# mala-lab/GGAD

Hardware: AMD Instinct MI355X
Metric: training nodes/sec (DGraph-Fin mini-batch GGAD) (higher is better)
Workload: dtype f32; 1 GPU; DGraph-Fin-size synthetic graph, mini-batch GGAD (GCN encoder); nodes=3700550, directed_entries=72953930, feat=17, emb=64, batch=150+50, graph=powerlaw(alpha=2.1,max_degree=2000), chunk_batches=150, hop2=ldsw, overlap=False, dense_cus=0, chain=0, dense_steps=XCD-resident chunk kernel: one launch per chunk on 28 CUs of one XCD, parallelism=dp1, optimizer=adam(lr=1e-3,wd=0.007), batch_streams=the reference's stream

## Files before the change

ggad_amd/csrc/hop2_ldsw.hip:

```cpp
#include <algorithm>
#include <atomic>
#include <climits>
#include <mutex>

#include "common.h"

namespace {

#ifdef GGAD_G2_PROF
struct G2Prof { unsigned long long a[8], t; };
#define G2_ARG , G2Prof &prof
#define G2_PASS , prof
#define G2_MARK(i) do { __builtin_amdgcn_sched_barrier(0); __builtin_amdgcn_s_waitcnt(0); const unsigned long long t_ = wall_clock64(); \
                        prof.a[i] += t_ - prof.t; prof.t = t_; __builtin_amdgcn_sched_barrier(0); } while (0)
#define TC_MARK(i) do { __syncthreads(); if (threadIdx.x == 0) { const unsigned long long t_ = wall_clock64(); tcp[i] += t_ - tct; tct = t_; } } while (0)
#else
#define G2_ARG
#define G2_PASS
#define G2_MARK(i)
#define TC_MARK(i)
#endif

constexpr int SLICE = 256;
constexpr int GRP_W = 10;
constexpr int ITEM_GRAB = 4;

__global__ void __launch_bounds__(256) k_tile_offsets(const int32_t *__restrict__ rowptr, const int32_t *__restrict__ col,
                                                      int64_t n_nodes, int n_tiles, int shift, int32_t *__restrict__ off) {
  const int64_t u = (int64_t)blockIdx.x * blockDim.x + threadIdx.x;
  if (u >= n_nodes) return;
  const int s = rowptr[u], e = rowptr[u + 1];
  int32_t *o = off + u * (n_tiles + 1);
  int t = 0;
  for (int i = s; i < e; ++i) {
    const int tile = col[i] >> shift;
    while (t <= tile) { o[t] = i - s; ++t; }
  }
  while (t <= n_tiles) { o[t] = e - s; ++t; }
}

__global__ void __launch_bounds__(256) k_tm_blocksum(const int32_t *__restrict__ off, int64_t n_nodes, int n_tiles, int32_t *__restrict__ bsum) {
  __shared__ int wsum[4][64];
  const int lane = lane_id(), w = threadIdx.x >> 6;
  const int NT1 = n_tiles + 1;
  const int64_t u0 = (int64_t)blockIdx.x * 256 + 64 * w;
  for (int t0 = 0; t0 < n_tiles; t0 += 64) {
    const int t = t0 + lane;
    int acc = 0;
    if (t < n_tiles)
      for (int i = 0; i < 64 && u0 + i < n_nodes; ++i) { const int32_t *o = off + (u0 + i) * NT1 + t; acc += o[1] - o[0]; }
    wsum[w][lane] = acc;
    __syncthreads();
    if (w == 0 && t < n_tiles) bsum[(int64_t)blockIdx.x * n_tiles + t] = wsum[0][lane] + wsum[1][lane] + wsum[2][lane] + wsum[3][lane];
    __syncthreads();
  }
}

__global__ void __launch_bounds__(1024) k_tm_scan(int32_t *__restrict__ bsum, int64_t n_blocks, int n_tiles, int32_t *__restrict__ tile_base) {
  extern __shared__ int tot[];
  for (int t = threadIdx.x; t < n_tiles; t += blockDim.x) {
    int run = 0;
    int64_t b = 0;
    for (; b + 8 <= n_blocks; b += 8) {
      int v[8];
#pragma unroll
      for (int q = 0; q < 8; ++q) v[q] = bsum[(b + q) * n_tiles + t];
#pragma unroll
      for (int q = 0; q < 8; ++q) { bsum[(b + q) * n_tiles + t] = run; run += v[q]; }
    }
    for (; b < n_blocks; ++b) { const int v = bsum[b * n_tiles + t]; bsum[b * n_tiles + t] = run; run += v; }
    tot[t] = run;
  }
  __syncthreads();
  if (threadIdx.x == 0) {
    int run = 0;
    for (int t = 0; t < n_tiles; ++t) { tile_base[t] = run; run += tot[t]; }
    tile_base[n_tiles] = run;
  }
}

__global__ void __launch_bounds__(256) k_tm_fill(const int32_t *__restrict__ rowptr, const int32_t *__restrict__ col,
                                                 const int32_t *__restrict__ off, int64_t n_nodes, int n_tiles,
                                                 const int32_t *__restrict__ bsum, const int32_t *__restrict__ tile_base,
                                                 int32_t *__restrict__ tile_start, int32_t *__restrict__ col_t) {
  __shared__ int wsum[4][64];
  const int lane = lane_id(), w = threadIdx.x >> 6;
  const int NT1 = n_tiles + 1;
  const int64_t u0 = (int64_t)blockIdx.x * 256 + 64 * w;
  for (int t0 = 0; t0 <= n_tiles; t0 += 64) {
    const int t = t0 + lane;
    int acc = 0;
    if (t < n_tiles)
      for (int i = 0; i < 64 && u0 + i < n_nodes; ++i) { const int32_t *o = off + (u0 + i) * NT1 + t; acc += o[1] - o[0]; }
    wsum[w][lane] = acc;
    __syncthreads();
    if (t < n_tiles) {
      int pos = tile_base[t] + bsum[(int64_t)blockIdx.x * n_tiles + t];
      for (int ww = 0; ww < w; ++ww) pos += wsum[ww][lane];
      for (int i = 0; i < 64 && u0 + i < n_nodes; ++i) {
        const int64_t u = u0 + i;
        const int32_t *o = off + u * NT1 + t;
        const int o0 = o[0], o1 = o[1];
        tile_start[u * NT1 + t] = pos;
        const int32_t *src = col + rowptr[u] + o0;
        for (int j = 0; j < o1 - o0; ++j) col_t[pos + j] = src[j];
        pos += o1 - o0;
      }
    } else if (t == n_tiles) {
      for (int i = 0; i < 64 && u0 + i < n_nodes; ++i) tile_start[(u0 + i) * NT1 + t] = 0;
    }
    __syncthreads();
  }
}

constexpr int TW_SHIFT = 15;
constexpr int TW_TILE = 1 << TW_SHIFT;
constexpr int TW_MAXOWN = 6144;
constexpr int TW_T = 1024;
constexpr int TW_BRK = 1536;

constexpr int TT_SLAB = 128;
__global__ void __launch_bounds__(256) k_seg_transpose(const int32_t *__restrict__ tile_off, const int32_t *__restrict__ tile_start,
                                                       int n_tiles, const int32_t *__restrict__ ent_own,
                                                       const int32_t *__restrict__ ent_col, int n_ents, int64_t seg_stride,
                                                       int32_t *__restrict__ seg_t, int skip) {
  __shared__ int tl[TT_SLAB][65];
  unsigned vbx, vgx;
  if (!ggad_vblock(skip, vbx, vgx)) return;
  const int p0 = vbx * 64;
  if (p0 >= n_ents) return;
  const int lane = lane_id(), wid = threadIdx.x >> 6;
  const int NT1 = n_tiles + 1;
  int u_l = 0, own_l = 0;
  if (p0 + lane < n_ents) { own_l = ent_own[p0 + lane] == p0 + lane ? 1 : 0; u_l = own_l ? ent_col[p0 + lane] : 0; }
  for (int which = 0; which < (tile_start ? 2 : 1); ++which) {
  const int32_t *table = which ? tile_start : tile_off;
  int32_t *plane = seg_t + (which ? (int64_t)NT1 * seg_stride : 0);
  for (int t0 = 0; t0 < NT1; t0 += TT_SLAB) {
    int v0[16], v1[16];
    const int c0 = min(t0 + lane, NT1 - 1), c1 = min(t0 + 64 + lane, NT1 - 1);
#pragma unroll
    for (int jj = 0; jj < 16; ++jj) {
      const int j = wid + 4 * jj;
      const int u = __shfl(u_l, j, GGAD_WAVE);
      const int32_t *row = table + (int64_t)u * NT1;
      v0[jj] = row[c0];
      v1[jj] = row[c1];
    }
#pragma unroll
    for (int jj = 0; jj < 16; ++jj) {
      const int j = wid + 4 * jj;
      const int own = __shfl(own_l, j, GGAD_WAVE);
      if (t0 + lane < NT1) tl[lane][j] = own ? v0[jj] : 0;
      if (t0 + 64 + lane < NT1) tl[64 + lane][j] = own ? v1[jj] : 0;
    }
    __syncthreads();
    const int nt = min(TT_SLAB, NT1 - t0);
    for (int idx = threadIdx.x; idx < nt * 64; idx += 256) {
      const int tt = idx >> 6, j = idx & 63;
      if (p0 + j < n_ents) plane[(int64_t)(t0 + tt) * seg_stride + p0 + j] = tl[tt][j];
    }
    __syncthreads();
  }
  }
}

__device__ __forceinline__ int block_excl_scan_1024(int v, int *warp_buf, int *total) {
  const int lane = lane_id(), wid = threadIdx.x >> 6;
  int inc = v;
#pragma unroll
  for (int off = 1; off < 64; off <<= 1) {
    const int t = __shfl_up(inc, off, 64);
    if (lane >= off) inc += t;
  }
  if (lane == 63) warp_buf[wid] = inc;
  __syncthreads();
  int base = 0, tot = 0;
#pragma unroll
  for (int w = 0; w < 16; ++w) { const int sv = warp_buf[w]; if (w < wid) base += sv; tot += sv; }
  __syncthreads();
  *total = tot;
  return base + inc - v;
}

__global__ void __launch_bounds__(TW_T) k_tile_counts(const int32_t *__restrict__ col, const int32_t *__restrict__ seg_t,
                                                      int64_t n_cap, const int32_t *__restrict__ own_rp,
                                                      const int32_t *__restrict__ batch_ent_ptr,
                                                      const int32_t *__restrict__ pw_base, uint16_t *__restrict__ pc, int n_tiles,
                                                      int n_batches, int32_t *__restrict__ counters, int skip, int tile_major) {
  extern __shared__ __attribute__((aligned(16))) uint32_t lds_u[];
  uint32_t *cnt = lds_u;
  int *offs = reinterpret_cast<int *>(lds_u + TW_TILE / 2);
  int *segbeg = offs + TW_MAXOWN + 1;
  int *dst = segbeg + TW_MAXOWN;
  int *brk = dst + TW_MAXOWN;
  __shared__ int wbuf[16];
  unsigned vbx, vgx;
  if (!ggad_vblock(skip, vbx, vgx)) return;
  int t, b;
  const bool class_map = (tile_major & 2) != 0;
  tile_major &= 1;
  if (class_map) {
    const int nx = skip < 0 ? 8 : 7, c = (int)(blockIdx.x & 7u);
    const int ci = c - ((skip >= 0 && c > skip) ? 1 : 0);
    const unsigned j = blockIdx.x >> 3;
    const int nt_c = ci < n_tiles ? (n_tiles - ci + nx - 1) / nx : 0;
    if (j >= (unsigned)nt_c * (unsigned)n_batches) return;
    t = ci + nx * (int)(j / (unsigned)n_batches);
    b = (int)(j % (unsigned)n_batches);
  } else {
    if (vbx >= (unsigned)n_tiles * (unsigned)n_batches) return;
    t = (int)(vbx % (unsigned)n_tiles); b = (int)(vbx / (unsigned)n_tiles);
  }
  const int o0 = batch_ent_ptr[b], o1 = batch_ent_ptr[b + 1];
  const int n_own_all = o1 - o0;
  const int32_t *seg_lo = seg_t + (int64_t)t * n_cap, *seg_hi = seg_lo + n_cap;
  const int32_t *seg_st = tile_major ? seg_t + (int64_t)(n_tiles + 1 + t) * n_cap : own_rp;
#ifdef GGAD_G2_PROF
  unsigned long long tcp[8] = {0, 0, 0, 0, 0, 0, 0, 0}, tct = wall_clock64();
#endif
  for (int i = threadIdx.x; i < TW_TILE / 2; i += TW_T) cnt[i] = 0u;
  constexpr int IPT = TW_MAXOWN / TW_T;
  const int n_slabs = (n_own_all + TW_MAXOWN - 1) / TW_MAXOWN;
  const bool one_slab = n_slabs == 1;
  constexpr int CACHE_IT = 16;
  int kc[CACHE_IT], dc[CACHE_IT];
  for (int pass = 0; pass < 2; ++pass) {
    for (int slab = 0; slab < n_slabs; ++slab) {
      const int ob0 = o0 + slab * TW_MAXOWN;
      const int n_own = min(TW_MAXOWN, o1 - ob0);
      if (pass == 0 || n_slabs > 1) {
        {
          int lo_[IPT], hi_[IPT], rp_[IPT], pb_[IPT];
#pragma unroll
          for (int q = 0; q < IPT; ++q) {
            const int i = min((int)threadIdx.x + q * TW_T, n_own - 1);
            lo_[q] = seg_lo[ob0 + i]; hi_[q] = seg_hi[ob0 + i]; rp_[q] = seg_st[ob0 + i]; pb_[q] = pw_base[ob0 + i];
          }
#pragma unroll
          for (int q = 0; q < IPT; ++q) {
            const int i = (int)threadIdx.x + q * TW_T;
            if (i < n_own) { offs[i] = hi_[q] - lo_[q]; segbeg[i] = rp_[q] + (tile_major ? 0 : lo_[q]); dst[i] = pb_[q] + lo_[q]; }
          }
        }
        __syncthreads();
        TC_MARK(0);
        int len[IPT];
        int mysum = 0;
#pragma unroll
        for (int q = 0; q < IPT; ++q) {
          const int i = threadIdx.x * IPT + q;
          len[q] = (i < n_own) ? offs[i] : 0;
          mysum += len[q];
        }
        __syncthreads();
        int P0;
        int ex = block_excl_scan_1024(mysum, wbuf, &P0);
#pragma unroll
        for (int q = 0; q < IPT; ++q) {
          const int i = threadIdx.x * IPT + q;
          if (i < n_own) offs[i] = ex;
          ex += len[q];
        }
        if (threadIdx.x == 0) offs[n_own] = P0;
        __syncthreads();
        TC_MARK(1);
      }
      const int P = offs[n_own];
      if (P > 0) {
        const int s0 = 1 << (31 - __clz(n_own));
        auto locate = [&](int pp, int &own, int &j) {
          int lo = 0;
          for (int st = s0; st > 0; st >>= 1) { const int m = lo + st; lo = (offs[min(m, n_own)] <= pp) ? m : lo; }
          own = lo; j = pp - offs[lo];
        };
        const int nblk = ((P - 1) >> 6) + 1;
        const bool use_brk = nblk + 1 <= TW_BRK;
        if (use_brk && (pass == 0 || n_slabs > 1)) {
          for (int b = threadIdx.x; b <= nblk; b += TW_T) {
            int own = n_own, j = 0;
            if (b < nblk) locate(min(64 * b, P - 1), own, j);
            brk[b] = own;
          }
          __syncthreads();
        }
        auto locate4 = [&](const int (&pp)[4], int (&own)[4], int (&j)[4]) {
          int lo[4] = {0, 0, 0, 0};
          int smax = s0;
          if (use_brk) {
            smax = 0;
#pragma unroll
            for (int q = 0; q < 4; ++q) {
              const int b = pp[q] >> 6;
              lo[q] = brk[b];
              const int w = brk[b + 1] - lo[q];
              smax = max(smax, w > 0 ? 1 << (31 - __clz(w)) : 0);
            }
          }
          for (int st = smax; st > 0; st >>= 1) {
#pragma unroll
            for (int q = 0; q < 4; ++q) { const int m = lo[q] + st; lo[q] = (offs[min(m, n_own)] <= pp[q]) ? m : lo[q]; }
          }
#pragma unroll
          for (int q = 0; q < 4; ++q) { own[q] = lo[q]; j[q] = pp[q] - offs[lo[q]]; }
        };
        int p_start = 0;
        if (one_slab) {
          if (pass == 0) {
#pragma unroll
            for (int g4 = 0; g4 < CACHE_IT; g4 += 4) {
              if (g4 * TW_T < P) {
                int pp[4], own[4], j[4];
#pragma unroll
                for (int q = 0; q < 4; ++q) pp[q] = min((g4 + q) * TW_T + (int)threadIdx.x, P - 1);
                locate4(pp, own, j);
#pragma unroll
                for (int q = 0; q < 4; ++q) {
                  kc[g4 + q] = col[segbeg[own[q]] + j[q]];
                  dc[g4 + q] = dst[own[q]] + j[q];
                }
              } else {
#pragma unroll
                for (int q = 0; q < 4; ++q) { kc[g4 + q] = 0; dc[g4 + q] = 0; }
              }
            }
#pragma unroll
            for (int it = 0; it < CACHE_IT; ++it) {
              const bool on = it * TW_T + (int)threadIdx.x < P;
              const int loc = kc[it] & (TW_TILE - 1);
              if (on) atomicAdd(&cnt[loc >> 1], 1u << ((loc & 1) << 4));
              kc[it] = on ? loc : -1;
            }
          } else {
#pragma unroll
            for (int it = 0; it < CACHE_IT; ++it)
              if (kc[it] >= 0) pc[dc[it]] = (uint16_t)((cnt[kc[it] >> 1] >> ((kc[it] & 1) << 4)) & 0xFFFFu);
          }
          p_start = CACHE_IT * TW_T;
          TC_MARK(2 + 2 * pass);
        }
        for (int p0 = p_start; p0 < P; p0 += 4 * TW_T) {
          int pp[4], own[4], j[4];
#pragma unroll
          for (int q = 0; q < 4; ++q) pp[q] = min(p0 + q * TW_T + (int)threadIdx.x, P - 1);
          locate4(pp, own, j);
          int k4[4];
#pragma unroll
          for (int q = 0; q < 4; ++q) k4[q] = col[segbeg[own[q]] + j[q]];
#pragma unroll
          for (int q = 0; q < 4; ++q) {
            if (p0 + q * TW_T + (int)threadIdx.x < P) {
              const int loc = k4[q] & (TW_TILE - 1);
              if (pass == 0) atomicAdd(&cnt[loc >> 1], 1u << ((loc & 1) << 4));
              else pc[(int64_t)dst[own[q]] + j[q]] = (uint16_t)((cnt[loc >> 1] >> ((loc & 1) << 4)) & 0xFFFFu);
            }
          }
        }
        TC_MARK(3 + 2 * pass);
      }
      __syncthreads();
    }
  }
#ifdef GGAD_G2_PROF
  if (threadIdx.x == 0) {
    unsigned long long *out = reinterpret_cast<unsigned long long *>(counters + GGAD_CTR_PROF) + 8;
    for (int k = 0; k < 6; ++k) atomicAdd(out + k, tcp[k]);
    atomicAdd(out + 6, 1ull);
  }
#endif
}

template <int G, int FT>
__device__ __forceinline__ void gather_slice(const int32_t *__restrict__ col, const float *__restrict__ feat, int F_rt, int stride,
                                             int s, int n0, int n1, float inv_sr, int n_occ, const int (&pb)[8],
                                             const uint16_t *__restrict__ pc, int lane, int k_first, float (&tot)[G] G2_ARG) {
  const int F = FT ? FT : F_rt;
  const int rpi = 64 / F;
  const int g = lane / F, f = lane - g * F;
  const bool act = g < rpi;
  const int gl = act ? g : rpi - 1;
  const char *fb = reinterpret_cast<const char *>(feat);
  const uint32_t rs = (uint32_t)stride * 4u, fo = (uint32_t)f * 4u;
  auto row_elem = [&](int kk) -> float { return *reinterpret_cast<const float *>(fb + ((uint32_t)kk * rs + fo)); };
  float acc[G];
#pragma unroll
  for (int j = 0; j < G; ++j) acc[j] = 0.0f;
  const int last = max(n1 - 1, 0);
  int k_nx = k_first;
  uint32_t c_nx[G];
  {
    const int ix = min(n0 + lane, last);
#pragma unroll
    for (int j = 0; j < G; ++j) c_nx[j] = pc[pb[j] + ix];
  }
  G2_MARK(2);
  for (int blk = n0; blk < n1; blk += 64) {
    const bool mine = blk + lane < n1;
    const int k = mine ? k_nx : 0;
    const int count = min(64, n1 - blk);
    float w[G];
    if (FT != 17) {
#pragma unroll
      for (int j = 0; j < G; ++j) w[j] = (j < n_occ && mine) ? inv_sr / sqrtf((float)c_nx[j]) : 0.0f;
    }
    if (FT == 17) {
      constexpr int IT = 22;
      float x[IT];
#pragma unroll
      for (int t = 0; t < IT; ++t) {
        const int kk = __shfl(k, (t * 3 + gl) & 63, GGAD_WAVE);
        x[t] = row_elem(kk);
      }
#pragma unroll
      for (int j = 0; j < G; ++j) w[j] = (j < n_occ && mine) ? inv_sr / sqrtf((float)c_nx[j]) : 0.0f;
      {
        const int ix = min(blk + 64 + lane, last);
        k_nx = col[s + ix];
#pragma unroll
        for (int j = 0; j < G; ++j) c_nx[j] = pc[pb[j] + ix];
      }
      G2_MARK(3);
#pragma unroll
      for (int t = 0; t < IT; ++t) {
        const int src = t * 3 + g;
        const float xv = (act && src < count) ? x[t] : 0.0f;
#pragma unroll
        for (int j = 0; j < G; ++j) {
          const float ws = __shfl(w[j], src & 63, GGAD_WAVE);
          acc[j] = fmaf((src < count) ? ws : 0.0f, xv, acc[j]);
        }
      }
      G2_MARK(4);
    } else {
      const int iters = (count + rpi - 1) / rpi;
      int tt = 0;
      for (; tt + 8 <= iters; tt += 8) {
        float x[8];
#pragma unroll
        for (int q = 0; q < 8; ++q) {
          const int kk = __shfl(k, ((tt + q) * rpi + gl) & 63, GGAD_WAVE);
          x[q] = row_elem(kk);
        }
#pragma unroll
        for (int q = 0; q < 8; ++q) {
          const int src = (tt + q) * rpi + g;
          const float xv = (act && src < count) ? x[q] : 0.0f;
#pragma unroll
          for (int j = 0; j < G; ++j) {
            const float ws = __shfl(w[j], src & 63, GGAD_WAVE);
            acc[j] = fmaf((src < count) ? ws : 0.0f, xv, acc[j]);
          }
        }
      }
      for (; tt < iters; ++tt) {
        const int src = tt * rpi + g;
        const int kk = __shfl(k, (tt * rpi + gl) & 63, GGAD_WAVE);
        const float xr = row_elem(kk);
        const float xv = (act && src < count) ? xr : 0.0f;
#pragma unroll
        for (int j = 0; j < G; ++j) {
          const float ws = __shfl(w[j], src & 63, GGAD_WAVE);
          acc[j] = fmaf((src < count) ? ws : 0.0f, xv, acc[j]);
        }
      }
      const int ix = min(blk + 64 + lane, last);
      k_nx = col[s + ix];
#pragma unroll
      for (int j = 0; j < G; ++j) c_nx[j] = pc[pb[j] + ix];
    }
  }
#pragma unroll
  for (int j = 0; j < G; ++j) {
    float t = acc[j];
    for (int q = 1; q < rpi; ++q) t += __shfl(acc[j], (lane + q * F) & 63, GGAD_WAVE);
    tot[j] = t;
  }
}

constexpr int MF_WS = 68;
constexpr int MF_LDS = 8 * MF_WS + 64;
typedef float mf4 __attribute__((ext_vector_type(4)));
typedef float mf2 __attribute__((ext_vector_type(2)));
typedef int mi4 __attribute__((ext_vector_type(4)));

template <int G>
__device__ __forceinline__ void gather_slice_mfma(const int32_t *__restrict__ col, const float *__restrict__ feat, int s, int n0, int n1,
                                                  float inv_sr, int n_occ, const int (&pb)[8], const uint16_t *__restrict__ pc,
                                                  int lane, float *lw, int k_first, float (&tot)[G] G2_ARG) {
  const int a = lane & 15, g = lane >> 4;
  const char *fb = reinterpret_cast<const char *>(feat) + a * 8;
  int *lids = reinterpret_cast<int *>(lw + 8 * MF_WS);
  const int aa = a < G ? a : 0;
  mf4 acc0 = {0.0f, 0.0f, 0.0f, 0.0f}, acc1 = {0.0f, 0.0f, 0.0f, 0.0f};
  const int last = max(n1 - 1, 0);
  int k_nx = k_first;
  uint32_t c_nx[G];
  {
    const int ix = min(n0 + lane, last);
#pragma unroll
    for (int j = 0; j < G; ++j) c_nx[j] = pc[pb[j] + ix];
  }
  G2_MARK(2);
  for (int blk = n0; blk < n1; blk += 64) {
    const bool mine = blk + lane < n1;
    lids[lane] = k_nx;
    __builtin_amdgcn_fence(__ATOMIC_RELEASE, "wavefront");
    __builtin_amdgcn_wave_barrier();
    int id[16];
#pragma unroll
    for (int c = 0; c < 4; ++c) {
      const mi4 iv = *reinterpret_cast<const mi4 *>(lids + 16 * g + 4 * c);
#pragma unroll
      for (int q = 0; q < 4; ++q) id[4 * c + q] = iv[q];
    }
    mf2 x[16];
#pragma unroll
    for (int i = 0; i < 16; ++i) x[i] = *reinterpret_cast<const mf2 *>(fb + ((uint32_t)id[i] << 7));
#pragma unroll
    for (int j = 0; j < G; ++j)
      lw[j * MF_WS + lane] = (j < n_occ && mine) ? inv_sr / sqrtf((float)c_nx[j]) : 0.0f;
    __builtin_amdgcn_fence(__ATOMIC_RELEASE, "wavefront");
    __builtin_amdgcn_wave_barrier();
    float wa[16];
#pragma unroll
    for (int c = 0; c < 4; ++c) {
      const mf4 wv = *reinterpret_cast<const mf4 *>(lw + aa * MF_WS + 16 * g + 4 * c);
#pragma unroll
      for (int q = 0; q < 4; ++q) wa[4 * c + q] = a < G ? wv[q] : 0.0f;
    }
    __builtin_amdgcn_wave_barrier();
    {
      const int ix = min(blk + 64 + lane, last);
      k_nx = col[s + ix];
#pragma unroll
      for (int j = 0; j < G; ++j) c_nx[j] = pc[pb[j] + ix];
    }
    G2_MARK(3);
#pragma unroll
    for (int i = 0; i < 16; ++i) {
      acc0 = __builtin_amdgcn_mfma_f32_16x16x4f32(wa[i], x[i].x, acc0, 0, 0, 0);
      acc1 = __builtin_amdgcn_mfma_f32_16x16x4f32(wa[i], x[i].y, acc1, 0, 0, 0);
    }
    G2_MARK(4);
  }
#pragma unroll
  for (int j = 0; j < G; ++j) {
    const int src = (lane >> 1) + 16 * (j >> 2);
    const float v0 = __shfl(acc0[j & 3], src & 63, GGAD_WAVE), v1 = __shfl(acc1[j & 3], src & 63, GGAD_WAVE);
    tot[j] = (lane & 1) ? v1 : v0;
  }
}

__device__ __forceinline__ int range_tile(int r, int n_tiles) { return (int)(((int64_t)r * n_tiles) / GGAD_RANGES); }

__global__ void __launch_bounds__(256) k_build_groups(const int32_t *__restrict__ ent_own, const int32_t *__restrict__ ent_col,
                                                      const int32_t *__restrict__ own_deg, int n_ents,
                                                      int32_t *__restrict__ node_head, const int32_t *__restrict__ own_next,
                                                      const int32_t *__restrict__ tile_off, int n_tiles,
                                                      int32_t *__restrict__ grp, int32_t *__restrict__ items,
                                                      int32_t *__restrict__ big, int32_t *__restrict__ gbnd,
                                                      int32_t *__restrict__ counters, int range_deg, int skip) {
  unsigned vbx, vgx;
  if (!ggad_vblock(skip, vbx, vgx)) return;
  const int e = vbx * 256 + threadIdx.x;
  const int lane = lane_id();
  int u = 0, m = 0, ng = 0, ns = 0, deg = 0;
  if (e < n_ents && ent_own[e] == e) {
    u = ent_col[e];
    if (node_head[u] == e + 1) {
      for (int cur = e + 1; cur != 0; cur = own_next[cur - 1]) ++m;
      ng = (m + 7) >> 3;
      deg = own_deg[e];
      ns = deg > range_deg ? GGAD_RANGES : (deg > SLICE ? (deg + SLICE - 1) / SLICE : 1);
    }
  }
  const bool is_big = deg > range_deg;
  const int c1 = is_big ? 0 : ng * ns, c2 = ns > 1 ? m * ns : 0, c3 = is_big ? ng : 0;
  int v0 = ng, v1 = c1, v2 = c2, v3 = c3;
#pragma unroll
  for (int off = 1; off < GGAD_WAVE; off <<= 1) {
    const int t0 = __shfl_up(v0, off, GGAD_WAVE), t1 = __shfl_up(v1, off, GGAD_WAVE), t2 = __shfl_up(v2, off, GGAD_WAVE),
              t3 = __shfl_up(v3, off, GGAD_WAVE);
    if (lane >= off) { v0 += t0; v1 += t1; v2 += t2; v3 += t3; }
  }
  __shared__ int wg_tot[4][5];
  const int wid = threadIdx.x >> 6;
  if (lane == GGAD_WAVE - 1) { wg_tot[0][wid] = v0; wg_tot[1][wid] = v1; wg_tot[2][wid] = v2; wg_tot[3][wid] = v3; }
  __syncthreads();
  if (threadIdx.x < 4) {
    const int k = threadIdx.x;
    int sum = 0;
    for (int w = 0; w < 4; ++w) { const int t = wg_tot[k][w]; wg_tot[k][w] = sum; sum += t; }
    int32_t *ctr = counters + (k == 0 ? GGAD_CTR_GROUPS : (k == 1 ? GGAD_CTR_ITEMS : (k == 2 ? GGAD_CTR_PART : GGAD_CTR_BIG)));
    wg_tot[k][4] = sum > 0 ? atomicAdd(ctr, sum) : 0;
  }
  __syncthreads();
  const int b0 = wg_tot[0][4] + wg_tot[0][wid], b1 = wg_tot[1][4] + wg_tot[1][wid], b2 = wg_tot[2][4] + wg_tot[2][wid],
            b3 = wg_tot[3][4] + wg_tot[3][wid];
  if (ng == 0) return;
  const int gbase = b0 + v0 - ng, ibase = b1 + v1 - c1, pbase = b2 + v2 - c2, bbase = b3 + v3 - c3;
  int bnd[GGAD_RANGES + 1];
  if (is_big) {
    const int32_t *row = tile_off + (int64_t)u * (n_tiles + 1);
#pragma unroll
    for (int r = 0; r <= GGAD_RANGES; ++r) bnd[r] = row[range_tile(r, n_tiles)];
  }
  int cur = e + 1;
  for (int g = 0; g < ng; ++g) {
    int32_t *rec = grp + (int64_t)(gbase + g) * GRP_W;
#pragma unroll
    for (int j = 0; j < 8; ++j) {
      int v = -1;
      if (cur != 0) { v = cur - 1; cur = own_next[v]; }
      rec[j] = v;
    }
    rec[8] = pbase + g * 8 * ns;
    rec[9] = ns;
    if (is_big) {
      big[bbase + g] = gbase + g;
      int32_t *bo = gbnd + (int64_t)(bbase + g) * (GGAD_RANGES + 1);
#pragma unroll
      for (int r = 0; r <= GGAD_RANGES; ++r) bo[r] = bnd[r];
    } else {
      for (int sl = 0; sl < ns; ++sl) {
        int32_t *it = items + (int64_t)(ibase + sl * ng + g) * 2;
        it[0] = gbase + g;
        it[1] = sl;
      }
    }
  }
  node_head[u] = 0;
}

template <int FT, bool MF>
__global__ void __launch_bounds__(256) k_gather2_items(const int32_t *__restrict__ col, const float *__restrict__ feat, int F_rt,
                                                       int stride, const int32_t *__restrict__ own_rp,
                                                       const int32_t *__restrict__ own_deg, const int32_t *__restrict__ pw_base,
                                                       const uint16_t *__restrict__ pc, const int32_t *__restrict__ grp,
                                                       const int32_t *__restrict__ items, const int32_t *__restrict__ big,
                                                       const int32_t *__restrict__ gbnd, int32_t *__restrict__ counters,
                                                       float *__restrict__ x2, float *__restrict__ part2, int affine, int take_cap, int skip) {
  static_assert(ITEM_GRAB == 4 && GRP_W <= 10, "lane layout of the metadata loads: 16 lanes per item of a grab (10, 11: range bounds)");
  unsigned vbx, vgx;
  if (!ggad_vblock(skip, vbx, vgx)) return;
  const int F = FT ? FT : F_rt;
  const int lane = lane_id();
  __shared__ __attribute__((aligned(16))) float mf_lds[MF ? 4 * MF_LDS : 4];
  float *lw = mf_lds + (MF ? (threadIdx.x >> 6) * MF_LDS : 0);
  const int n_small = counters[GGAD_CTR_ITEMS], n_big = counters[GGAD_CTR_BIG];
  const int q_l = lane >> 4, r_l = lane & 15;
  unsigned xcc;
  asm volatile("s_getreg_b32 %0, hwreg(HW_REG_XCC_ID)" : "=s"(xcc));
  xcc &= GGAD_RANGES - 1;
  if (!affine) xcc = (vbx / GGAD_RANGES) & (GGAD_RANGES - 1);
  const int n_waves_all = (int)vgx * 4;
#ifdef GGAD_G2_PROF
  G2Prof prof = {};
  const unsigned long long t_begin = wall_clock64();
  prof.t = t_begin;
#endif
  for (int ph = 0; ph <= GGAD_RANGES; ++ph) {
    const int cls = ph == 0 ? (int)xcc : (ph == 1 ? GGAD_RANGES : (int)((xcc + ph - 1) & (GGAD_RANGES - 1)));
    const bool bigc = cls < GGAD_RANGES;
    const int n_items = bigc ? n_big : n_small;
    if (n_items == 0) continue;
    int32_t *cursor = counters + (bigc ? GGAD_CTR_RANGE0 + cls * GGAD_CTR_STRIDE : GGAD_CTR_CURSOR);
    const int n_waves = ph == 0 ? max(n_waves_all / GGAD_RANGES, 1) : n_waves_all;
    int seen = 0;
    if (ph != 0) {
      seen = __hip_atomic_load(cursor, __ATOMIC_RELAXED, __HIP_MEMORY_SCOPE_AGENT);
      if (seen >= n_items) continue;
    }
  for (;;) {
    const int rem = n_items - seen;
    int take = (rem / (2 * n_waves)) & ~(ITEM_GRAB - 1);
    take = take < ITEM_GRAB ? ITEM_GRAB : (take > take_cap ? take_cap : take);
    int first = 0;
    if (lane == 0) first = atomicAdd(cursor, take);
    first = __builtin_amdgcn_readfirstlane(first);
    G2_MARK(0);
    if (first >= n_items) break;
    seen = first + take;
    const int last = min(n_items, first + take);
#pragma unroll 1
    for (int base = first; base < last; base += ITEM_GRAB) {
    const bool it_ok = base + q_l < last;
    int iv;
    if (bigc) iv = r_l == 0 ? (it_ok ? big[base + q_l] : 0) : cls;
    else iv = (it_ok && r_l < 2) ? items[(int64_t)(base + q_l) * 2 + r_l] : 0;
    const int bv = (bigc && it_ok && (r_l == 10 || r_l == 11)) ? gbnd[(int64_t)(base + q_l) * (GGAD_RANGES + 1) + cls + (r_l - 10)] : 0;
    const int gi_l = __shfl(iv, q_l * 16, GGAD_WAVE);
    const int rv = (it_ok && r_l < GRP_W) ? grp[(int64_t)gi_l * GRP_W + r_l] : -1;
    const int pbv = (r_l < 8 && rv >= 0) ? pw_base[rv] : 0;
    const int rpv = (it_ok && r_l == 0) ? own_rp[rv] : 0;
    const int dgv = (it_ok && r_l == 0) ? own_deg[rv] : 0;
    G2_MARK(1);
    auto item_span = [&](int q, int &s_, int &n0_, int &n1_, int &deg_) {
      s_ = __builtin_amdgcn_readlane(rpv, q * 16);
      deg_ = __builtin_amdgcn_readlane(dgv, q * 16);
      const int sl_ = __builtin_amdgcn_readlane(iv, q * 16 + 1);
      n0_ = bigc ? __builtin_amdgcn_readlane(bv, q * 16 + 10) : sl_ * SLICE;
      n1_ = bigc ? __builtin_amdgcn_readlane(bv, q * 16 + 11) : min(deg_, n0_ + SLICE);
    };
    auto first_ids = [&](int s_, int n0_, int n1_) { return col[s_ + min(n0_ + lane, max(n1_ - 1, 0))]; };
    int k_ahead = 0;
    { int s_, a_, b_, d_; item_span(0, s_, a_, b_, d_); k_ahead = first_ids(s_, a_, b_); }
#pragma unroll 1
    for (int q = 0; q < ITEM_GRAB; ++q) {
      if (base + q >= last) break;
      int e[8], pb[8];
      int n = 0;
#pragma unroll
      for (int j = 0; j < 8; ++j) {
        e[j] = __builtin_amdgcn_readlane(rv, q * 16 + j);
        pb[j] = __builtin_amdgcn_readlane(pbv, q * 16 + j);
        n += e[j] >= 0 ? 1 : 0;
      }
      const int pbase = __builtin_amdgcn_readlane(rv, q * 16 + 8), ns = __builtin_amdgcn_readlane(rv, q * 16 + 9);
      const int sl = __builtin_amdgcn_readlane(iv, q * 16 + 1);
      int s, n0, n1, deg;
      item_span(q, s, n0, n1, deg);
      const float inv_sr = 1.0f / sqrtf((float)deg);
      const int k_first = k_ahead;
      if (q + 1 < ITEM_GRAB && base + q + 1 < last) {
        int s_, a_, b_, d_;
        item_span(q + 1, s_, a_, b_, d_);
        k_ahead = first_ids(s_, a_, b_);
      }
      float tot[8];
      if (MF) {
        if (n == 1) { float t1[1]; gather_slice_mfma<1>(col, feat, s, n0, n1, inv_sr, n, pb, pc, lane, lw, k_first, t1 G2_PASS); tot[0] = t1[0]; }
        else if (n == 2) { float t2[2]; gather_slice_mfma<2>(col, feat, s, n0, n1, inv_sr, n, pb, pc, lane, lw, k_first, t2 G2_PASS); tot[0] = t2[0]; tot[1] = t2[1]; }
        else if (n <= 4) { float t4[4]; gather_slice_mfma<4>(col, feat, s, n0, n1, inv_sr, n, pb, pc, lane, lw, k_first, t4 G2_PASS);
#pragma unroll
          for (int j = 0; j < 4; ++j) tot[j] = t4[j]; }
        else gather_slice_mfma<8>(col, feat, s, n0, n1, inv_sr, n, pb, pc, lane, lw, k_first, tot G2_PASS);
      } else
      if (n == 1) { float t1[1]; gather_slice<1, FT>(col, feat, F, stride, s, n0, n1, inv_sr, n, pb, pc, lane, k_first, t1 G2_PASS); tot[0] = t1[0]; }
      else if (n == 2) { float t2[2]; gather_slice<2, FT>(col, feat, F, stride, s, n0, n1, inv_sr, n, pb, pc, lane, k_first, t2 G2_PASS); tot[0] = t2[0]; tot[1] = t2[1]; }
      else if (n <= 4) { float t4[4]; gather_slice<4, FT>(col, feat, F, stride, s, n0, n1, inv_sr, n, pb, pc, lane, k_first, t4 G2_PASS);
#pragma unroll
        for (int j = 0; j < 4; ++j) tot[j] = t4[j]; }
      else gather_slice<8, FT>(col, feat, F, stride, s, n0, n1, inv_sr, n, pb, pc, lane, k_first, tot G2_PASS);
#pragma unroll
      for (int j = 0; j < 8; ++j) {
        if (j < n && lane < F) {
          if (ns == 1) x2[(int64_t)e[j] * F + lane] = (deg == 0) ? inv_sr * 0.0f : tot[j];
          else part2[((int64_t)pbase + (int64_t)j * ns + sl) * F + lane] = tot[j];
        }
      }
      G2_MARK(5);
    }
    }
  }
  }
#ifdef GGAD_G2_PROF
  if (lane == 0) {
    prof.a[6] = wall_clock64() - t_begin;
    unsigned long long *out = reinterpret_cast<unsigned long long *>(counters + GGAD_CTR_PROF);
    for (int k = 0; k < 7; ++k) atomicAdd(out + k, prof.a[k]);
  }
#endif
}

__global__ void __launch_bounds__(256) k_gather2_combine(const int32_t *__restrict__ grp, const int32_t *__restrict__ counters,
                                                         const float *__restrict__ part2, int F, float *__restrict__ x2, int skip) {
  unsigned vbx, vgx;
  if (!ggad_vblock(skip, vbx, vgx)) return;
  const int lane = lane_id();
  const int n_groups = counters[GGAD_CTR_GROUPS];
  const int rpi = 64 / F;
  const int g = lane / F, f = lane - g * F;
  for (int gi = vbx * 4 + (threadIdx.x >> 6); gi < n_groups; gi += vgx * 4) {
    const int rv = (lane < GRP_W) ? grp[(int64_t)gi * GRP_W + lane] : -1;
    const int ns = __builtin_amdgcn_readlane(rv, 9);
    if (ns <= 1) continue;
    const int pbase = __builtin_amdgcn_readlane(rv, 8);
    for (int j0 = 0; j0 < 8; j0 += rpi) {
      const int j = j0 + g;
      const int ej = __shfl(rv, j & 7, GGAD_WAVE);
      if (g < rpi && j < 8 && ej >= 0) {
        float acc = 0.0f;
#pragma unroll 4
        for (int sl = 0; sl < ns; ++sl) acc += part2[((int64_t)pbase + (int64_t)j * ns + sl) * F + f];
        x2[(int64_t)ej * F + f] = acc;
      }
    }
  }
}

__global__ void __launch_bounds__(256) k_gather2_w(const int32_t *__restrict__ col, const float *__restrict__ feat, int F, int stride,
                                                   const int32_t *__restrict__ ent_own, int n_ents,
                                                   const int32_t *__restrict__ own_rp, const int32_t *__restrict__ own_deg,
                                                   const int32_t *__restrict__ pw_base, const uint16_t *__restrict__ pc,
                                                   float *__restrict__ x2, int skip) {
  unsigned vbx, vgx;
  if (!ggad_vblock(skip, vbx, vgx)) return;
  const int e0 = vbx * 4 + (threadIdx.x >> 6);
  if (e0 >= n_ents || ent_own[e0] != e0) return;
  const int lane = lane_id();
  const int s = own_rp[e0];
  const int deg = own_deg[e0];
  const int pb0 = pw_base[e0];
  const float inv_sr = 1.0f / sqrtf((float)deg);
  if (F <= 64) {
    const int pb[8] = {pb0, 0, 0, 0, 0, 0, 0, 0};
    float total = 0.0f;
#ifdef GGAD_G2_PROF
    G2Prof prof = {};
#endif
    for (int n0 = 0; n0 < deg; n0 += SLICE) {
      float t1[1];
      const int kf = col[s + min(n0 + lane, max(min(deg, n0 + SLICE) - 1, 0))];
      if (F == 17) gather_slice<1, 17>(col, feat, F, stride, s, n0, min(deg, n0 + SLICE), inv_sr, 1, pb, pc, lane, kf, t1 G2_PASS);
      else gather_slice<1, 0>(col, feat, F, stride, s, n0, min(deg, n0 + SLICE), inv_sr, 1, pb, pc, lane, kf, t1 G2_PASS);
      total += t1[0];
    }
    if (deg == 0) total = inv_sr * 0.0f;
    if (lane < F) x2[(int64_t)e0 * F + lane] = total;
    return;
  }
  for (int fbase = 0; fbase < F; fbase += 64) {
    const int fw = min(64, F - fbase);
    float total = 0.0f;
    for (int n0 = 0; n0 < deg; n0 += SLICE) {
      const int n1 = min(deg, n0 + SLICE);
      float acc = 0.0f;
      for (int blk = n0; blk < n1; blk += 64) {
        const int idx = blk + lane;
        int k = 0;
        float w = 0.0f;
        if (idx < n1) { k = col[s + idx]; w = inv_sr / sqrtf((float)pc[pb0 + idx]); }
        const int count = min(64, n1 - blk);
        for (int t = 0; t < count; ++t) {
          const int kk = __shfl(k, t, GGAD_WAVE);
          const float ws = __shfl(w, t, GGAD_WAVE);
          const float x = lane < fw ? feat[(int64_t)kk * stride + fbase + lane] : 0.0f;
          acc = fmaf(ws, x, acc);
        }
      }
      total += acc;
    }
    if (deg == 0) total = inv_sr * 0.0f;
    if (lane < fw) x2[(int64_t)e0 * F + fbase + lane] = total;
  }
}

std::atomic<int> g_mfma_batches{[] { const char *e = getenv("GGAD_GATHER_MFMA_BATCHES"); return e ? atoi(e) : 0; }()};
std::atomic<int> g_range_deg{[] { const char *e = getenv("GGAD_RANGE_DEG"); return e ? atoi(e) : 0; }()};

}

int ggad_int_range_deg() { return g_range_deg.load() > 0 ? std::max(g_range_deg.load(), GGAD_RANGE_DEG) : INT32_MAX; }

int ggad_int_ldsw_hop2(const ggad_mb_plan *P, const ggad_plan_view &V, hipStream_t st, hipEvent_t ev0, hipEvent_t ev1) {
  if (V.n_ents == 0 || V.n_batches == 0) return GGAD_OK;
  const int n_tiles = (int)((P->n_nodes + TW_TILE - 1) >> TW_SHIFT);
  const int skip = P->xcd_skip >= 0 && P->xcd_skip < 8 ? P->xcd_skip : -1;
  const bool tile_major = P->tile_start != nullptr && P->col_t != nullptr;
  k_seg_transpose<<<dim3(ggad_skip_grid((unsigned)((V.n_ents + 63) / 64), skip)), dim3(256), 0, st>>>(
      P->tile_off, tile_major ? P->tile_start : nullptr, n_tiles, P->ent_own, P->ent_col, V.n_ents, V.seg_stride, P->seg_t, skip);
  const size_t lds = (size_t)(TW_TILE / 2) * 4 + (size_t)(3 * TW_MAXOWN + 1) * 4 + (size_t)TW_BRK * 4;
  {
    static std::mutex mu;
    static int state[64] = {};
    int dev = 0;
    if (hipGetDevice(&dev) != hipSuccess || dev < 0 || dev >= 64) return GGAD_E_INVALID;
    std::lock_guard<std::mutex> lock(mu);
    if (state[dev] == 0) {
      const bool ok = hipFuncSetAttribute((const void *)k_tile_counts, hipFuncAttributeMaxDynamicSharedMemorySize, (int)lds) == hipSuccess;
      (void)hipGetLastError();
      state[dev] = ok ? 1 : -1;
    }
    if (state[dev] != 1) { ggad_set_error(hipErrorInvalidValue, "mb_plan_build: this device cannot give k_tile_counts its LDS"); return GGAD_E_LAUNCH; }
  }
  if (P->ev_tile0) (void)hipEventRecord(static_cast<hipEvent_t>(P->ev_tile0), st);
  static const int tc_map = [] { const char *e = getenv("GGAD_TC_MAP"); return e ? atoi(e) : -1; }();
  const bool class_map = tc_map >= 0 ? tc_map != 0 : tile_major;
  const unsigned tc_grid = class_map ? 8u * (unsigned)((n_tiles + (skip < 0 ? 8 : 7) - 1) / (skip < 0 ? 8 : 7)) * (unsigned)V.n_batches
                                      : ggad_skip_grid((unsigned)n_tiles * (unsigned)V.n_batches, skip);
  k_tile_counts<<<dim3(tc_grid), dim3(TW_T), lds, st>>>(tile_major ? P->col_t : P->col, P->seg_t, V.seg_stride, P->own_rp, V.batch_ent_ptr,
                                                        P->pw_base, P->pc, n_tiles, V.n_batches, P->counters, skip, (tile_major ? 1 : 0) | (class_map ? 2 : 0));
  if (P->ev_tile1) (void)hipEventRecord(static_cast<hipEvent_t>(P->ev_tile1), st);
  if (ev0) (void)hipEventRecord(ev0, st);
  const int F = P->feat_dim;
  if (P->node_major && F <= 64) {
    const int range_deg = ggad_int_range_deg();
    static const int affine = [] { const char *e = getenv("GGAD_RANGE_AFFINE"); return e ? atoi(e) : 1; }();
    int32_t *big = P->items + 2 * (int64_t)P->item_cap, *gbnd = P->items + 3 * (int64_t)P->item_cap;
    k_build_groups<<<dim3(ggad_skip_grid((unsigned)((V.n_ents + 255) / 256), skip)), dim3(256), 0, st>>>(
        P->ent_own, P->ent_col, P->own_deg, V.n_ents, P->node_head, P->own_next, P->tile_off, n_tiles, P->grp, P->items, big, gbnd,
        P->counters, range_deg, skip);
    const int64_t max_items = (int64_t)V.n_ents + (V.pair_bound > 0 ? V.pair_bound : P->pair_cap) / SLICE;
    static const int env_wg = [] { const char *e = getenv("GGAD_G2_WG_PER_CU"); return e ? atoi(e) : 0; }();
    static const int env_cap = [] { const char *e = getenv("GGAD_G2_TAKE_CAP"); return e ? atoi(e) : 0; }();
    const bool small_launch = V.n_batches <= 32;
    const int wg_per_cu = env_wg > 0 ? env_wg : (small_launch ? 3 : 4);
    const int take_cap = env_cap > 0 ? env_cap : (small_launch ? 8 : 12);
    const unsigned wgs = (unsigned)std::min<int64_t>((max_items + 4 * ITEM_GRAB - 1) / (4 * ITEM_GRAB), 256 * wg_per_cu);
    if (F == 17 && P->feat_stride == 32 && V.n_batches >= g_mfma_batches.load())
      k_gather2_items<17, true><<<dim3(ggad_skip_grid(wgs, skip)), dim3(256), 0, st>>>(P->col, P->feat, F, P->feat_stride, P->own_rp, P->own_deg,
                                                                                       P->pw_base, P->pc, P->grp, P->items, big, gbnd, P->counters,
                                                                                       P->x2, P->part2, affine, take_cap, skip);
    else if (F == 17)
      k_gather2_items<17, false><<<dim3(ggad_skip_grid(wgs, skip)), dim3(256), 0, st>>>(P->col, P->feat, F, P->feat_stride, P->own_rp, P->own_deg,
                                                                                 P->pw_base, P->pc, P->grp, P->items, big, gbnd, P->counters,
                                                                                 P->x2, P->part2, affine, take_cap, skip);
    else
      k_gather2_items<0, false><<<dim3(ggad_skip_grid(wgs, skip)), dim3(256), 0, st>>>(P->col, P->feat, F, P->feat_stride, P->own_rp, P->own_deg,
                                                                                P->pw_base, P->pc, P->grp, P->items, big, gbnd, P->counters,
                                                                                P->x2, P->part2, affine, take_cap, skip);
    const unsigned cg = (unsigned)std::min<int64_t>(((int64_t)V.n_ents + 3) / 4, 16384);
    k_gather2_combine<<<dim3(ggad_skip_grid(cg, skip)), dim3(256), 0, st>>>(P->grp, P->counters, P->part2, F, P->x2, skip);
  } else {
    k_gather2_w<<<dim3(ggad_skip_grid((unsigned)((V.n_ents + 3) / 4), skip)), dim3(256), 0, st>>>(
        P->col, P->feat, F, P->feat_stride, P->ent_own, V.n_ents, P->own_rp, P->own_deg, P->pw_base, P->pc, P->x2, skip);
  }
  if (ev1) (void)hipEventRecord(ev1, st);
  GGAD_CHECK_LAUNCH("mb_plan_build (ldsw 2-hop)");
  return GGAD_OK;
}

extern "C" {

int ggad_mb_ldsw_tile_shift(void) { return TW_SHIFT; }
int ggad_mb_ldsw_max_owners(void) { return TW_MAXOWN; }
int32_t ggad_mb_slice_len(void) { return SLICE; }
int32_t ggad_mb_group_words(void) { return GRP_W; }
int ggad_mb_set_gather_options(int32_t mfma_min_batches, int32_t range_deg) {
  if (mfma_min_batches >= 0) g_mfma_batches.store(mfma_min_batches);
  if (range_deg >= 0) g_range_deg.store(range_deg);
  return GGAD_OK;
}
int32_t ggad_mb_item_words(void) { return 3 + GGAD_RANGES + 1; }
int32_t ggad_mb_plan_counter_elems(void) { return GGAD_PLAN_COUNTERS; }
int64_t ggad_mb_tile_offsets_elems(int64_t n_nodes, int32_t tile_shift) {
  return n_nodes * (((n_nodes + (1LL << tile_shift) - 1) >> tile_shift) + 1);
}
int64_t ggad_mb_ldsw_seg_elems(int64_t n_nodes, int64_t n_entries_cap) {
  return 2 * (((n_nodes + TW_TILE - 1) >> TW_SHIFT) + 1) * ((n_entries_cap + 63) / 64 * 64);
}

int ggad_mb_tile_offsets(const int32_t *rowptr, const int32_t *col, int64_t n_nodes, int32_t tile_shift, int32_t *tile_off,
                         ggad_stream_t stream) {
  GGAD_REQUIRE(rowptr && col && tile_off && n_nodes >= 0 && tile_shift >= 8 && tile_shift <= 24);
  if (n_nodes == 0) return GGAD_OK;
  const int n_tiles = (int)((n_nodes + (1LL << tile_shift) - 1) >> tile_shift);
  k_tile_offsets<<<dim3((unsigned)((n_nodes + 255) / 256)), dim3(256), 0, as_stream(stream)>>>(rowptr, col, n_nodes, n_tiles,
                                                                                               tile_shift, tile_off);
  GGAD_CHECK_LAUNCH("mb_tile_offsets");
  return GGAD_OK;
}


int64_t ggad_mb_tile_major_workspace_elems(int64_t n_nodes, int32_t tile_shift) {
  if (n_nodes < 0 || tile_shift < 8 || tile_shift > 24) return 0;
  const int64_t n_tiles = (n_nodes + (1LL << tile_shift) - 1) >> tile_shift;
  return ((n_nodes + 255) / 256) * n_tiles + n_tiles + 1;
}

int ggad_mb_tile_major(const int32_t *rowptr, const int32_t *col, int64_t n_nodes, int32_t tile_shift, const int32_t *tile_off,
                       int32_t *tile_start, int32_t *col_t, int32_t *workspace, ggad_stream_t stream) {
  GGAD_REQUIRE(rowptr && col && tile_off && tile_start && col_t && workspace && n_nodes >= 0 && tile_shift >= 8 && tile_shift <= 24);
  if (n_nodes == 0) return GGAD_OK;
  const int n_tiles = (int)((n_nodes + (1LL << tile_shift) - 1) >> tile_shift);
  const int64_t n_blocks = (n_nodes + 255) / 256;
  GGAD_REQUIRE(n_tiles <= 16384 && n_blocks < (1LL << 31));
  hipStream_t st = as_stream(stream);
  int32_t *bsum = workspace, *tile_base = workspace + n_blocks * n_tiles;
  k_tm_blocksum<<<dim3((unsigned)n_blocks), dim3(256), 0, st>>>(tile_off, n_nodes, n_tiles, bsum);
  k_tm_scan<<<dim3(1), dim3(1024), (size_t)n_tiles * sizeof(int), st>>>(bsum, n_blocks, n_tiles, tile_base);
  k_tm_fill<<<dim3((unsigned)n_blocks), dim3(256), 0, st>>>(rowptr, col, tile_off, n_nodes, n_tiles, bsum, tile_base, tile_start, col_t);
  GGAD_CHECK_LAUNCH("mb_tile_major");
  return GGAD_OK;
}

}
```

Baseline: 3.306 million nodes/s.

## Fuse adjacent same-slice item pairs into one 16-row MFMA gather pass

When two consecutive work items share the same neighbor slice (same row start, degree and slice offset) and the first has a full group of 8 occurrences, the MFMA gather now handles both in one pass. It uses up to 16 A-rows, so the column ids and feature rows are loaded once instead of twice. LDS per wave grows to hold 16 weight rows, and a launch-bounds occupancy hint of 4 is added for the MFMA variant. The new path is on by default and can be disabled with an environment variable. It adds template instantiations and register pressure, and only helps when such pairs occur.

```diff
diff --git a/ggad_amd/csrc/hop2_ldsw.hip b/ggad_amd/csrc/hop2_ldsw.hip
--- a/ggad_amd/csrc/hop2_ldsw.hip
+++ b/ggad_amd/csrc/hop2_ldsw.hip
@@ -478,27 +478,34 @@
 }
 
 constexpr int MF_WS = 68;
-constexpr int MF_LDS = 8 * MF_WS + 64;
+constexpr int MF_ROWS = 16;
+constexpr int MF_LDS = MF_ROWS * MF_WS + 64;
 typedef float mf4 __attribute__((ext_vector_type(4)));
 typedef float mf2 __attribute__((ext_vector_type(2)));
 typedef int mi4 __attribute__((ext_vector_type(4)));
 
 template <int G>
 __device__ __forceinline__ void gather_slice_mfma(const int32_t *__restrict__ col, const float *__restrict__ feat, int s, int n0, int n1,
-                                                  float inv_sr, int n_occ, const int (&pb)[8], const uint16_t *__restrict__ pc,
+                                                  float inv_sr, int n_occ, const int (&pb)[MF_ROWS], const uint16_t *__restrict__ pc,
                                                   int lane, float *lw, int k_first, float (&tot)[G] G2_ARG) {
+  static_assert(G >= 1 && G <= MF_ROWS, "one row of A per occurrence");
   const int a = lane & 15, g = lane >> 4;
   const char *fb = reinterpret_cast<const char *>(feat) + a * 8;
-  int *lids = reinterpret_cast<int *>(lw + 8 * MF_WS);
+  int *lids = reinterpret_cast<int *>(lw + MF_ROWS * MF_WS);
   const int aa = a < G ? a : 0;
   mf4 acc0 = {0.0f, 0.0f, 0.0f, 0.0f}, acc1 = {0.0f, 0.0f, 0.0f, 0.0f};
   const int last = max(n1 - 1, 0);
   int k_nx = k_first;
+  const char *pcb = reinterpret_cast<const char *>(pc);
+  auto count_at = [&](int j, int ix) -> uint32_t {
+    if constexpr (G <= 8) return pc[pb[j] + ix];
+    else return *reinterpret_cast<const uint16_t *>(pcb + (int64_t)pb[j] * 2 + (uint32_t)(ix << 1));
+  };
   uint32_t c_nx[G];
   {
     const int ix = min(n0 + lane, last);
 #pragma unroll
-    for (int j = 0; j < G; ++j) c_nx[j] = pc[pb[j] + ix];
+    for (int j = 0; j < G; ++j) c_nx[j] = count_at(j, ix);
   }
   G2_MARK(2);
   for (int blk = n0; blk < n1; blk += 64) {
@@ -533,7 +540,7 @@
       const int ix = min(blk + 64 + lane, last);
       k_nx = col[s + ix];
 #pragma unroll
-      for (int j = 0; j < G; ++j) c_nx[j] = pc[pb[j] + ix];
+      for (int j = 0; j < G; ++j) c_nx[j] = count_at(j, ix);
     }
     G2_MARK(3);
 #pragma unroll
@@ -633,13 +640,13 @@
 }
 
 template <int FT, bool MF>
-__global__ void __launch_bounds__(256) k_gather2_items(const int32_t *__restrict__ col, const float *__restrict__ feat, int F_rt,
+__global__ void __launch_bounds__(256, MF ? 4 : 1) k_gather2_items(const int32_t *__restrict__ col, const float *__restrict__ feat, int F_rt,
                                                        int stride, const int32_t *__restrict__ own_rp,
                                                        const int32_t *__restrict__ own_deg, const int32_t *__restrict__ pw_base,
                                                        const uint16_t *__restrict__ pc, const int32_t *__restrict__ grp,
                                                        const int32_t *__restrict__ items, const int32_t *__restrict__ big,
                                                        const int32_t *__restrict__ gbnd, int32_t *__restrict__ counters,
-                                                       float *__restrict__ x2, float *__restrict__ part2, int affine, int take_cap, int skip) {
+                                                       float *__restrict__ x2, float *__restrict__ part2, int affine, int take_cap, int skip, int pair) {
   static_assert(ITEM_GRAB == 4 && GRP_W <= 10, "lane layout of the metadata loads: 16 lanes per item of a grab (10, 11: range bounds)");
   unsigned vbx, vgx;
   if (!ggad_vblock(skip, vbx, vgx)) return;
@@ -708,7 +715,7 @@
 #pragma unroll 1
     for (int q = 0; q < ITEM_GRAB; ++q) {
       if (base + q >= last) break;
-      int e[8], pb[8];
+      int e[8], pb[MF ? MF_ROWS : 8];
       int n = 0;
 #pragma unroll
       for (int j = 0; j < 8; ++j) {
@@ -722,13 +729,61 @@
       item_span(q, s, n0, n1, deg);
       const float inv_sr = 1.0f / sqrtf((float)deg);
       const int k_first = k_ahead;
-      if (q + 1 < ITEM_GRAB && base + q + 1 < last) {
+      bool fuse = false;
+      if (MF && pair && !bigc && n == 8 && q + 1 < ITEM_GRAB && base + q + 1 < last) {
         int s_, a_, b_, d_;
         item_span(q + 1, s_, a_, b_, d_);
+        fuse = s_ == s && d_ == deg && a_ == n0;
+      }
+      const int q_nx = q + (fuse ? 2 : 1);
+      if (q_nx < ITEM_GRAB && base + q_nx < last) {
+        int s_, a_, b_, d_;
+        item_span(q_nx, s_, a_, b_, d_);
         k_ahead = first_ids(s_, a_, b_);
       }
+      if constexpr (MF) {
+        if (fuse) {
+          int e2[8];
+          int m = 0;
+#pragma unroll
+          for (int j = 0; j < 8; ++j) {
+            e2[j] = __builtin_amdgcn_readlane(rv, q * 16 + 16 + j);
+            pb[8 + j] = __builtin_amdgcn_readlane(pbv, q * 16 + 16 + j);
+            m += e2[j] >= 0 ? 1 : 0;
+          }
+          const int pbase2 = __builtin_amdgcn_readlane(rv, q * 16 + 16 + 8), ns2 = __builtin_amdgcn_readlane(rv, q * 16 + 16 + 9);
+          float t16[16];
+          if (m == 1) { float t[9]; gather_slice_mfma<9>(col, feat, s, n0, n1, inv_sr, 9, pb, pc, lane, lw, k_first, t G2_PASS);
+#pragma unroll
+            for (int j = 0; j < 9; ++j) t16[j] = t[j]; }
+          else if (m == 2) { float t[10]; gather_slice_mfma<10>(col, feat, s, n0, n1, inv_sr, 10, pb, pc, lane, lw, k_first, t G2_PASS);
+#pragma unroll
+            for (int j = 0; j < 10; ++j) t16[j] = t[j]; }
+          else if (m <= 4) { float t[12]; gather_slice_mfma<12>(col, feat, s, n0, n1, inv_sr, 8 + m, pb, pc, lane, lw, k_first, t G2_PASS);
+#pragma unroll
+            for (int j = 0; j < 12; ++j) t16[j] = t[j]; }
+          else gather_slice_mfma<16>(col, feat, s, n0, n1, inv_sr, 8 + m, pb, pc, lane, lw, k_first, t16 G2_PASS);
+#pragma unroll
+          for (int j = 0; j < 8; ++j) {
+            if (lane < F) {
+              if (ns == 1) x2[(int64_t)e[j] * F + lane] = (deg == 0) ? inv_sr * 0.0f : t16[j];
+              else part2[((int64_t)pbase + (int64_t)j * ns + sl) * F + lane] = t16[j];
+            }
+          }
+#pragma unroll
+          for (int j = 0; j < 8; ++j) {
+            if (j < m && lane < F) {
+              if (ns2 == 1) x2[(int64_t)e2[j] * F + lane] = (deg == 0) ? inv_sr * 0.0f : t16[8 + j];
+              else part2[((int64_t)pbase2 + (int64_t)j * ns2 + sl) * F + lane] = t16[8 + j];
+            }
+          }
+          G2_MARK(5);
+          ++q;
+          continue;
+        }
+      }
       float tot[8];
-      if (MF) {
+      if constexpr (MF) {
         if (n == 1) { float t1[1]; gather_slice_mfma<1>(col, feat, s, n0, n1, inv_sr, n, pb, pc, lane, lw, k_first, t1 G2_PASS); tot[0] = t1[0]; }
         else if (n == 2) { float t2[2]; gather_slice_mfma<2>(col, feat, s, n0, n1, inv_sr, n, pb, pc, lane, lw, k_first, t2 G2_PASS); tot[0] = t2[0]; tot[1] = t2[1]; }
         else if (n <= 4) { float t4[4]; gather_slice_mfma<4>(col, feat, s, n0, n1, inv_sr, n, pb, pc, lane, lw, k_first, t4 G2_PASS);
@@ -887,6 +942,7 @@
   if (P->node_major && F <= 64) {
     const int range_deg = ggad_int_range_deg();
     static const int affine = [] { const char *e = getenv("GGAD_RANGE_AFFINE"); return e ? atoi(e) : 1; }();
+    static const int pair = [] { const char *e = getenv("GGAD_G2_PAIR"); return e ? atoi(e) : 1; }();
     int32_t *big = P->items + 2 * (int64_t)P->item_cap, *gbnd = P->items + 3 * (int64_t)P->item_cap;
     k_build_groups<<<dim3(ggad_skip_grid((unsigned)((V.n_ents + 255) / 256), skip)), dim3(256), 0, st>>>(
         P->ent_own, P->ent_col, P->own_deg, V.n_ents, P->node_head, P->own_next, P->tile_off, n_tiles, P->grp, P->items, big, gbnd,
@@ -901,15 +957,15 @@
     if (F == 17 && P->feat_stride == 32 && V.n_batches >= g_mfma_batches.load())
       k_gather2_items<17, true><<<dim3(ggad_skip_grid(wgs, skip)), dim3(256), 0, st>>>(P->col, P->feat, F, P->feat_stride, P->own_rp, P->own_deg,
                                                                                        P->pw_base, P->pc, P->grp, P->items, big, gbnd, P->counters,
-                                                                                       P->x2, P->part2, affine, take_cap, skip);
+                                                                                       P->x2, P->part2, affine, take_cap, skip, pair);
     else if (F == 17)
       k_gather2_items<17, false><<<dim3(ggad_skip_grid(wgs, skip)), dim3(256), 0, st>>>(P->col, P->feat, F, P->feat_stride, P->own_rp, P->own_deg,
                                                                                  P->pw_base, P->pc, P->grp, P->items, big, gbnd, P->counters,
-                                                                                 P->x2, P->part2, affine, take_cap, skip);
+                                                                                 P->x2, P->part2, affine, take_cap, skip, pair);
     else
       k_gather2_items<0, false><<<dim3(ggad_skip_grid(wgs, skip)), dim3(256), 0, st>>>(P->col, P->feat, F, P->feat_stride, P->own_rp, P->own_deg,
                                                                                 P->pw_base, P->pc, P->grp, P->items, big, gbnd, P->counters,
-                                                                                P->x2, P->part2, affine, take_cap, skip);
+                                                                                P->x2, P->part2, affine, take_cap, skip, pair);
     const unsigned cg = (unsigned)std::min<int64_t>(((int64_t)V.n_ents + 3) / 4, 16384);
     k_gather2_combine<<<dim3(ggad_skip_grid(cg, skip)), dim3(256), 0, st>>>(P->grp, P->counters, P->part2, F, P->x2, skip);
   } else {
```

Result: slower. 3.235 million nodes/s (-2.1%).
